# aymenboudhina/Multimodal_VQVAE_compression_audio_tactile

Measured on AMD Instinct MI355X. Metric: encode+VQ+decode token-frames/sec (1 frame = 13.33 ms of paired 24 kHz audio+tactile), higher is better.
Workload: dtype f32

## Files before the change

### multimodal_vqvae_compression_audio_tactile_amd/csrc/conv1d_mfma.hpp

```cpp
#pragma once
#include <hip/hip_runtime.h>
#include <stdio.h>
#include <stdlib.h>
#include <type_traits>
#include "det_math.hpp"
#include "kernels_small.hpp"

namespace mvq {

struct ConvArgs;
inline bool conv_dma_rows_ok(const ConvArgs& a);

__device__ __attribute__((aligned(16))) static const float g_zero16[4] = {0.0f, 0.0f, 0.0f, 0.0f};

int prof_begin(const char* kernel_name, double flops, hipStream_t s);
void prof_end(int idx, hipStream_t s);
bool prof_enabled();

typedef float f32x16 __attribute__((ext_vector_type(16)));
typedef float f32x4 __attribute__((ext_vector_type(4)));

struct ConvArgs {
    const float* x;
    const float* wp;
// ... 137 lines not shown
                     : "=&s"(keep) : "v"(off[0]), "v"(off[1]), "v"(off[2]), "v"(off[3]), "v"(off[4]), "v"(off[5]), "v"(off[6]), [base] "s"(base), [dst] "s"(dst), [inc] "n"(INC) : "memory", "scc");
    else
        asm volatile(MVQ_DMA_HEAD MVQ_DMAU_FIRST(1) MVQ_DMAU_NEXT(2) MVQ_DMAU_NEXT(3) MVQ_DMAU_NEXT(4) MVQ_DMAU_NEXT(5) MVQ_DMAU_NEXT(6) MVQ_DMAU_NEXT(7) MVQ_DMAU_NEXT(8) MVQ_DMA_TAIL
                     : "=&s"(keep) : "v"(off[0]), "v"(off[1]), "v"(off[2]), "v"(off[3]), "v"(off[4]), "v"(off[5]), "v"(off[6]), "v"(off[7]), [base] "s"(base), [dst] "s"(dst), [inc] "n"(INC) : "memory", "scc");
}
__device__ __forceinline__ void lds_dma_masked_uni(unsigned off, unsigned long long base, unsigned dst, unsigned long long mask)
{
    unsigned keep;
    unsigned long long keep_exec;
    asm volatile("s_mov_b64 %1, exec\n\ts_mov_b64 exec, %[mask]\n\t"
                 "s_mov_b32 %0, m0\n\ts_mov_b32 m0, %[dst]\n\ts_nop 0\n\tglobal_load_lds_dwordx4 %2, %[base]\n\ts_mov_b32 m0, %0\n\t"
                 "s_mov_b64 exec, %1"
                 : "=&s"(keep), "=&s"(keep_exec) : "v"(off), [base] "s"(base), [dst] "s"(dst), [mask] "s"(mask) : "memory");
}

__device__ __forceinline__ unsigned long long dma_scalar_base(const float* p)
{
    const unsigned long long v = (unsigned long long)p;
    const unsigned lo = __builtin_amdgcn_readfirstlane((unsigned)v), hi = __builtin_amdgcn_readfirstlane((unsigned)(v >> 32));
    unsigned long long s = ((unsigned long long)hi << 32) | lo;
    asm volatile("s_nop 4" : "+s"(s));
    return s;
}

template <int KS, int STRIDE, int DIL, int BM, int XP, int MT, int NT, int NS, int BASE = 0>
struct AsmOperandLoop {
    template <int S, int I>
    static __device__ __forceinline__ void load_a(float (&av)[MT], unsigned a_addr)
    {
        if constexpr (I < MT) {
            av[I] = lds_read_imm<BASE + (2 * S * BM + I * 32) * 4>(a_addr);
            load_a<S, I + 1>(av, a_addr);
        }
    }
    template <int S, int J>
    static __device__ __forceinline__ void load_b(float (&bv)[NT], unsigned b_same, unsigned b_cross)
    {
        if constexpr (J < NT) {
            constexpr int k0 = 2 * S;
            constexpr int off0 = (k0 / KS) * XP + (k0 % KS) * DIL;
            constexpr bool cross = ((k0 + 1) / KS) != (k0 / KS);
            bv[J] = lds_read_imm<BASE + (off0 + J * 32 * STRIDE) * 4>(cross ? b_cross : b_same);
            load_b<S, J + 1>(bv, b_same, b_cross);
        }
    }
    template <int S>
    static __device__ __forceinline__ void load_step(float (&av)[MT], float (&bv)[NT], unsigned a_addr, unsigned b_same, unsigned b_cross)
    {
        load_a<S, 0>(av, a_addr);
        load_b<S, 0>(bv, b_same, b_cross);
    }
    static __device__ __forceinline__ void mfma_step(f32x16_t (&acc)[MT][NT], const float (&av)[MT], const float (&bv)[NT])
    {
#pragma unroll
        for (int i = 0; i < MT; ++i)
#pragma unroll
            for (int j = 0; j < NT; ++j)
                acc[i][j] = __builtin_amdgcn_mfma_f32_32x32x2f32(av[i], bv[j], acc[i][j], 0, 0, 0);
    }
    template <int S>
    static __device__ __forceinline__ void run_from(f32x16_t (&acc)[MT][NT], float (&av0)[MT], float (&bv0)[NT], float (&av1)[MT],
                                                    float (&bv1)[NT], unsigned a_addr, unsigned b_same, unsigned b_cross)
    {
        if constexpr (S < NS) {
            if constexpr (S + 1 < NS) {
                if constexpr ((S + 1) % 2 == 0) load_step<S + 1>(av0, bv0, a_addr, b_same, b_cross);
                else load_step<S + 1>(av1, bv1, a_addr, b_same, b_cross);
            }
            constexpr int PW = (S + 1 < NS) ? MT + NT : 0;
            __builtin_amdgcn_sched_barrier(0);
            if constexpr (S % 2 == 0) lgkm_wait_step<PW, MT, NT>(av0, bv0);
            else lgkm_wait_step<PW, MT, NT>(av1, bv1);
            __builtin_amdgcn_sched_barrier(0);
            if constexpr (S % 2 == 0) mfma_step(acc, av0, bv0);
            else mfma_step(acc, av1, bv1);
            __builtin_amdgcn_sched_barrier(0);
            run_from<S + 1>(acc, av0, bv0, av1, bv1, a_addr, b_same, b_cross);
        }
    }
};

constexpr int cgcd(int a, int b) { return b == 0 ? a : cgcd(b, a % b); }

template <int KS, int STRIDE, int DIL, int CK, int MT, int NT, int WAVES_M, int WAVES_N, int UPS>
struct ConvCfg {
    static constexpr int BM = 32 * MT * WAVES_M;
    static constexpr int BN = 32 * NT * WAVES_N;
    static constexpr int KC = CK * KS;
    static constexpr int XT = (BN - 1) * STRIDE + (KS - 1) * DIL + 1;
    static constexpr bool XALIGNED = (KS == 1 && STRIDE == 1);
    static constexpr int XV = XALIGNED ? (XT + 3) / 4 : (XT + 3 + 3) / 4;
    static constexpr int XTP = XV * 4 + 4;
    static constexpr int W_FLOATS = KC * BM;
    static constexpr int X_FLOATS = CK * XTP;
    static constexpr int STAGE_FLOATS = 2 * (W_FLOATS + X_FLOATS);
    static constexpr int BNP = BN + 4;
    static constexpr int CT_FLOATS = BM * BNP;
    static constexpr int EH = ((UPS == 0 || 32 % (UPS ? UPS : 1) == 0) && MT % 2 == 0 && CT_FLOATS > STAGE_FLOATS) ? 2 : 1;
    static constexpr int CTH_FLOATS = CT_FLOATS / EH;
    static constexpr int QPR = BN / 4;
    static constexpr int CQ = cgcd(QPR, 64 * WAVES_M * WAVES_N);
    static constexpr int JN = QPR / CQ;
    static constexpr int RSTEP = (64 * WAVES_M * WAVES_N) / CQ;
    static constexpr bool REG_GEOM = (UPS == 0) && (32 % RSTEP == 0);
    static constexpr int TB_FLOATS = REG_GEOM ? 2 * BM : 0;
    static constexpr int EPI_FLOATS = CTH_FLOATS + TB_FLOATS;
    static constexpr int EPI_FLOATS_FUSE = CT_FLOATS + TB_FLOATS;
    static constexpr int LDS_FLOATS = STAGE_FLOATS > EPI_FLOATS ? STAGE_FLOATS : EPI_FLOATS;
    static constexpr bool FOUR_WAVES = WAVES_M * WAVES_N == 4;
    static constexpr bool RING_FITS = (size_t)3 * (KC * BM + CK * XV * 4) * 4 <= 64 * 1024;
    static constexpr int MIN_WPE = (FOUR_WAVES && LDS_FLOATS * 4 <= 53 * 1024 && !(WAVES_N == 4 && NT == 2) && RING_FITS && MT * NT <= 4) ? 3
                                                                                                                : (WAVES_M * WAVES_N) / 2;
    static constexpr int LDS_FLOATS_FUSE = STAGE_FLOATS > EPI_FLOATS_FUSE ? STAGE_FLOATS : EPI_FLOATS_FUSE;
    static constexpr int MIN_WPE_FUSE = (FOUR_WAVES && (LDS_FLOATS_FUSE + 5 * BM) * 4 * 3 <= 160 * 1024) ? 3 : (WAVES_M * WAVES_N) / 2;
    static constexpr int XV4 = XV * 4;
    static constexpr int DMA_STAGE_FLOATS = W_FLOATS + CK * XV4;
    static constexpr int DMA_NV = DMA_STAGE_FLOATS / 4;
    static constexpr int DMA_NU = (DMA_NV + 64 * WAVES_M * WAVES_N - 1) / (64 * WAVES_M * WAVES_N);
    static constexpr int LDS_FLOATS_DMA = 3 * DMA_STAGE_FLOATS > EPI_FLOATS ? 3 * DMA_STAGE_FLOATS : EPI_FLOATS;
    static constexpr int LDS_FLOATS_FUSE_DMA = 3 * DMA_STAGE_FLOATS > EPI_FLOATS_FUSE ? 3 * DMA_STAGE_FLOATS : EPI_FLOATS_FUSE;
    static constexpr int W_VEC = W_FLOATS / 4;
    static constexpr int NTHR = 64 * WAVES_M * WAVES_N;
    static constexpr int W_PER_THREAD = (W_VEC + NTHR - 1) / NTHR;
    static constexpr int XV_TOTAL = CK * XV;
    static constexpr int XV_PER_THREAD = (XV_TOTAL + NTHR - 1) / NTHR;
    static constexpr int XS_TOTAL = CK * XT;
    static constexpr int XS_PER_THREAD = (XS_TOTAL + NTHR - 1) / NTHR;
    static constexpr int XREGS = (4 * XV_PER_THREAD > XS_PER_THREAD) ? 4 * XV_PER_THREAD : XS_PER_THREAD;
    static_assert(WAVES_M * WAVES_N == 4 || WAVES_M * WAVES_N == 8, "block is 4 or 8 waves");
    static_assert(KC % 2 == 0, "chunk K must be even (32x32x2 MFMA)");
    static_assert(BM % 4 == 0, "float4 weight staging");
};

template <int KS, int STRIDE, int DIL, int CK, int MT, int NT, int WAVES_M, int WAVES_N, int UPS, bool VEC>
struct ConvTile {
    using C = ConvCfg<KS, STRIDE, DIL, CK, MT, NT, WAVES_M, WAVES_N, UPS>;
    const float* wp; const float* xb; const float* Al;
    float* Ws; float* Xs;
    int tid, Tin, Cin, Mpad, m0, t_in0, g_al;
    bool snake_in;

    __device__ __forceinline__ void load_chunk(int chunk, f32x4 (&wreg)[C::W_PER_THREAD], f32x4 (&xv)[C::XV_PER_THREAD], float (&xs)[C::XS_PER_THREAD]) const
    {
        const int ci0 = chunk * CK;
        const float* wsrc = wp + (size_t)ci0 * KS * Mpad + m0;
#pragma unroll
        for (int u = 0; u < C::W_PER_THREAD; ++u) {
            int v = tid + u * C::NTHR;
            if (C::W_VEC % C::NTHR != 0) v = v < C::W_VEC ? v : C::W_VEC - 1;
            const int row = v / (C::BM / 4);
            const int c4 = v - row * (C::BM / 4);
            wreg[u] = *reinterpret_cast<const f32x4*>(wsrc + (size_t)row * Mpad + c4 * 4);
        }
        if (VEC) {
#pragma unroll
            for (int u = 0; u < C::XV_PER_THREAD; ++u) {
                int e = tid + u * C::NTHR;
                if (C::XV_TOTAL % C::NTHR != 0) e = e < C::XV_TOTAL ? e : C::XV_TOTAL - 1;
                const int cl = e / C::XV;
                const int v = e - cl * C::XV;
                const int g = g_al + 4 * v;
                const bool ok = g >= 0 && g < Tin;
                const int gc = ok ? g : 0;
                xv[u] = *reinterpret_cast<const f32x4*>(xb + (size_t)(ci0 + cl) * Tin + gc);
            }
        } else {
#pragma unroll
            for (int u = 0; u < C::XS_PER_THREAD; ++u) {
                int e = tid + u * C::NTHR;
                if (C::XS_TOTAL % C::NTHR != 0) e = e < C::XS_TOTAL ? e : C::XS_TOTAL - 1;
                const int cl = e / C::XT;
                const int xi = e - cl * C::XT;
                const int g = t_in0 + xi;
                const bool ok = g >= 0 && g < Tin;
                const int gc = ok ? g : 0;
                xs[u] = xb[(size_t)(ci0 + cl) * Tin + gc];
            }
        }
    }

    __device__ __forceinline__ void store_chunk(int chunk, int buf, const f32x4 (&wreg)[C::W_PER_THREAD],
                                                const f32x4 (&xv)[C::XV_PER_THREAD],
                                                const float (&xs)[C::XS_PER_THREAD]) const
    {
        const int ci0 = chunk * CK;
        float* wdst = Ws + buf * C::W_FLOATS;
        float* xdst = Xs + buf * C::X_FLOATS;
#pragma unroll
        for (int u = 0; u < C::W_PER_THREAD; ++u) {
            const int v = tid + u * C::NTHR;
            if (C::W_VEC % C::NTHR == 0 || v < C::W_VEC) *reinterpret_cast<f32x4*>(wdst + v * 4) = wreg[u];
        }
        if (VEC) {
#pragma unroll
            for (int u = 0; u < C::XV_PER_THREAD; ++u) {
                const int e = tid + u * C::NTHR;
                const int ec = (C::XV_TOTAL % C::NTHR != 0 && e >= C::XV_TOTAL) ? C::XV_TOTAL - 1 : e;
                const int cl = ec / C::XV;
                const int v = ec - cl * C::XV;
                const int g = g_al + 4 * v;
                const bool ok = g >= 0 && g < Tin;
                f32x4 q = xv[u];
                if (!ok) q = f32x4{0.0f, 0.0f, 0.0f, 0.0f};
                if (snake_in) {
                    const float al = Al[ci0 + cl], inv = Al[Cin + ci0 + cl];
                    q.x = det_snake(q.x, al, inv); q.y = det_snake(q.y, al, inv);
                    q.z = det_snake(q.z, al, inv); q.w = det_snake(q.w, al, inv);
                }
                if (C::XV_TOTAL % C::NTHR == 0 || e < C::XV_TOTAL)
                    *reinterpret_cast<f32x4*>(xdst + cl * C::XTP + 4 * v) = q;
            }
        } else {
#pragma unroll
            for (int u = 0; u < C::XS_PER_THREAD; ++u) {
                const int e = tid + u * C::NTHR;
                const int ec = (C::XS_TOTAL % C::NTHR != 0 && e >= C::XS_TOTAL) ? C::XS_TOTAL - 1 : e;
                const int cl = ec / C::XT;
                const int xi = ec - cl * C::XT;
                const int g = t_in0 + xi;
                float q = (g >= 0 && g < Tin) ? xs[u] : 0.0f;
                if (snake_in) q = det_snake(q, Al[ci0 + cl], Al[Cin + ci0 + cl]);
                if (C::XS_TOTAL % C::NTHR == 0 || e < C::XS_TOTAL) xdst[cl * C::XTP + xi] = q;
            }
        }
    }
};

template <int KS, int STRIDE, int DIL, int CK, int MT, int NT, int WAVES_M, int WAVES_N, int UPS, bool VEC, bool FUSE>
__device__ __forceinline__ void conv1d_mfma_body(const ConvArgs& a)
{
    using C = ConvCfg<KS, STRIDE, DIL, CK, MT, NT, WAVES_M, WAVES_N, UPS>;
    extern __shared__ __attribute__((aligned(16))) float smem[];
    float* const Ws = smem;
    float* const Xs = smem + 2 * C::W_FLOATS;
    float* const Ep = smem + (FUSE ? (a.dma ? C::LDS_FLOATS_FUSE_DMA : C::LDS_FLOATS_FUSE) : (a.dma ? C::LDS_FLOATS_DMA : C::LDS_FLOATS));
    constexpr int EP_MID = 2;
    float* const Al = Ep + 3 * C::BM;

    const int tid = threadIdx.x;
    const int lane = tid & 63;
    const int wave = tid >> 6;
    const int wm = wave / WAVES_N;
    const int wn = wave % WAVES_N;
    const int l31 = lane & 31;
    const int h = lane >> 5;

    int bx = blockIdx.x, by = blockIdx.y;
    if (a.row_fast) {
        const int xcd = bx & 7, j = bx >> 3;
        by = j % a.row_fast;
        bx = (j / a.row_fast) * 8 + xcd;
        if (bx >= a.n_tiles * a.B) return;
    }
    const int b = bx / a.n_tiles;
    const int tile_n = bx - b * a.n_tiles;
    const int n0 = a.n_base + tile_n * C::BN;
    const int m0 = by * C::BM;
    const int t_in0 = n0 * STRIDE - a.pad;
    const int g_al = t_in0 & ~3;
    const int shift = VEC ? (t_in0 - g_al) : 0;
    const int Cin = a.Cin;
    const int n_chunks = Cin / CK;
    const bool snake_in = a.alpha_in != nullptr;

    if (snake_in) {
        for (int c = tid; c < Cin; c += C::NTHR) {
            const float al = a.alpha_in[c];
            Al[c] = al;
            Al[Cin + c] = 1.0f / (al + 1e-9f);
        }
    }
    for (int r = tid; r < C::BM; r += C::NTHR) {
        int m = m0 + r;
        m = m < a.Mrows ? m : a.Mrows - 1;
        const int ch = m / (UPS ? UPS : 1);
        const float* tabs[4] = {a.alpha_out, a.y2 ? a.alpha2 : nullptr, FUSE ? a.alpha_mid : (a.dsn_src ? a.dsn_alpha : nullptr), nullptr};
#pragma unroll
        for (int k = 0; k < 3; ++k) {
            Ep[k * C::BM + r] = tabs[k] ? 1.0f / (tabs[k][ch] + 1e-9f) : 1.0f;
        }
    }

    ConvTile<KS, STRIDE, DIL, CK, MT, NT, WAVES_M, WAVES_N, UPS, VEC> tile;
    tile.wp = a.wp; tile.xb = a.x + (size_t)b * Cin * a.Tin; tile.Al = Al; tile.Ws = Ws; tile.Xs = Xs;
    tile.tid = tid; tile.Tin = a.Tin; tile.Cin = Cin; tile.Mpad = a.Mpad; tile.m0 = m0; tile.t_in0 = t_in0;
    tile.g_al = g_al; tile.snake_in = snake_in;

    f32x16 acc[MT][NT];
#pragma unroll
    for (int i = 0; i < MT; ++i)
#pragma unroll
        for (int j = 0; j < NT; ++j)
#pragma unroll
            for (int r = 0; r < 16; ++r) acc[i][j][r] = 0.0f;

    f32x4 wreg[C::W_PER_THREAD];
    f32x4 xv[C::XV_PER_THREAD];
    float xs[C::XS_PER_THREAD];

    constexpr int D_SAME = DIL;
    constexpr int D_CROSS = C::XTP - (KS - 1) * DIL;
    const int a_base = h * C::BM + wm * (MT * 32) + l31;
    const int b_base = (wn * (NT * 32) + l31) * STRIDE + shift;
    const int b_same = b_base + h * D_SAME;
    const int b_cross = b_base + h * D_CROSS;

    constexpr int NS = C::KC / 2;
    auto mfma_chunk = [&](int buf) __attribute__((always_inline)) {
        const float* wsrc = Ws + buf * C::W_FLOATS + a_base;
        const float* xs_same = Xs + buf * C::X_FLOATS + b_same;
        const float* xs_cross = Xs + buf * C::X_FLOATS + b_cross;
        float av[2][MT], bv[2][NT];
        auto load_step = [&](int st, int pb) __attribute__((always_inline)) {
            const int k0 = 2 * st;
            const int off0 = (k0 / KS) * C::XTP + (k0 % KS) * DIL;
            const bool cross = ((k0 + 1) / KS) != (k0 / KS);
            const float* xsp = cross ? xs_cross : xs_same;
#pragma unroll
            for (int i = 0; i < MT; ++i) av[pb][i] = wsrc[k0 * C::BM + i * 32];
#pragma unroll
            for (int j = 0; j < NT; ++j) bv[pb][j] = xsp[off0 + j * 32 * STRIDE];
        };
        load_step(0, 0);
#pragma unroll
        for (int s = 0; s < NS; ++s) {
            const int pb = s & 1;
            if (s + 1 < NS) load_step(s + 1, (s + 1) & 1);
#pragma unroll
            for (int i = 0; i < MT; ++i)
#pragma unroll
                for (int j = 0; j < NT; ++j)
                    acc[i][j] = __builtin_amdgcn_mfma_f32_32x32x2f32(av[pb][i], bv[pb][j], acc[i][j], 0, 0, 0);
            __builtin_amdgcn_sched_group_barrier(0x100, MT + NT, 0);
            __builtin_amdgcn_sched_group_barrier(0x008, MT * NT, 0);
        }
    };

    constexpr bool DMA_FITS = FUSE ? ((size_t)C::LDS_FLOATS_FUSE_DMA + 3 * C::BM) * 4 * 2 <= 160 * 1024 : (size_t)C::LDS_FLOATS_DMA * 4 <= 64 * 1024;
    bool use_dma = false;
    if constexpr (VEC && DMA_FITS) use_dma = a.dma != 0;
    if (use_dma) {
      if constexpr (VEC && DMA_FITS) {
        constexpr int NU = C::DMA_NU;
        constexpr int XP = C::XV4;
        constexpr int D_CROSS_D = XP - (KS - 1) * DIL;
        const int bd_same = b_base + h * D_SAME;
        const int bd_cross = b_base + h * D_CROSS_D;
        const unsigned lds0 = (unsigned)(size_t)smem;
        const int wave_u = __builtin_amdgcn_readfirstlane(wave);
        using AL = AsmOperandLoop<KS, STRIDE, DIL, C::BM, XP, MT, NT, NS>;
        auto chunk_rt = [&](int stage, auto&& issue) __attribute__((always_inline)) {
            const unsigned sb = lds0 + (unsigned)(stage * C::DMA_STAGE_FLOATS * 4);
            const unsigned a_addr = sb + (unsigned)(a_base * 4);
            const unsigned b_s = sb + (unsigned)((C::W_FLOATS + bd_same) * 4), b_c = sb + (unsigned)((C::W_FLOATS + bd_cross) * 4);
            float av0[MT], bv0[NT], av1[MT], bv1[NT];
            AL::template load_step<0>(av0, bv0, a_addr, b_s, b_c);
            issue();
            AL::template run_from<0>(acc, av0, bv0, av1, bv1, a_addr, b_s, b_c);
        };
        constexpr int NW = WAVES_M * WAVES_N;
        constexpr int XPC = CK * C::XV;
        constexpr int WI_W = (C::W_VEC + 63) / 64, WI_X = (XPC + 63) / 64;
// ... 72 lines not shown
                    st_n2 = st_n2 == 2 ? 0 : st_n2 + 1;
                }
            };
            dma_uni(0);
            if (n_chunks > 1) dma_uni(1);
            const int my_issue = (WI_W - wave_u + NW - 1) / NW + (WI_X - xw + NW - 1) / NW;
            if ((WI_W + WI_X) % NW != 0 && my_issue > NI_MIN) k_loop_uni(std::integral_constant<int, NI_MIN + 1>{});
            else k_loop_uni(std::integral_constant<int, NI_MIN>{});
          }
        } else {
        const float* src[NU];
        bool live[NU];
        long long step_b[NU];
#pragma unroll
        for (int u = 0; u < NU; ++u) {
            const int p = tid + u * C::NTHR;
            live[u] = p < C::DMA_NV;
            if (p < C::W_VEC) {
                const int row = p / (C::BM / 4), c4 = p - row * (C::BM / 4);
                src[u] = a.wp + (size_t)row * a.Mpad + m0 + c4 * 4;
                step_b[u] = (long long)CK * KS * a.Mpad;
            } else {
                const int q = (p < C::DMA_NV ? p : C::DMA_NV - 1) - C::W_VEC;
                const int cl = q / C::XV, v = q - cl * C::XV;
                const int g = g_al + 4 * v;
                bool ok = g >= 0 && g < a.Tin;
                const float* sp = tile.xb + (size_t)cl * a.Tin + g;
                long long st = (long long)CK * a.Tin;
                if (a.vp_seg) {
                    const int gg = ok ? g : 0;
                    const int seg = (int)__umulhi((unsigned)gg, a.vp_magic_in), pos = gg - seg * a.vp_per_in;
                    const int item = b * a.vp_seg + seg;
                    ok = ok && pos < a.vp_valid_in && item < a.vp_btrue;
                    sp = a.x + ((size_t)(ok ? item : 0) * a.Cin + cl) * a.vp_tin_phys + (ok ? pos : 0);
                    st = (long long)CK * a.vp_tin_phys;
                }
                src[u] = ok ? sp : g_zero16;
                step_b[u] = ok ? st : 0;
            }
        }
        const int n_issue = (NU - 1) * C::NTHR + wave_u * 64 < C::DMA_NV ? NU : NU - 1;
        constexpr int NFULL = C::DMA_NV / C::NTHR < NU ? C::DMA_NV / C::NTHR : NU;
        auto dma_chunk = [&](int stage) __attribute__((always_inline)) {
            const unsigned dst0 = lds0 + (unsigned)(stage * C::DMA_STAGE_FLOATS * 4) + (unsigned)(wave_u * 64 * 16);
            if constexpr (NFULL > 0) lds_dma_burst<NFULL, C::NTHR * 16>(src, dst0);
#pragma unroll
            for (int u = NFULL; u < NU; ++u) {
                if (live[u]) lds_dma_burst<1, C::NTHR * 16>(src + u, dst0 + (unsigned)(u * C::NTHR * 16));
            }
#pragma unroll
            for (int u = 0; u < NU; ++u) src[u] += step_b[u];
        };
        dma_chunk(0);
        if (n_chunks > 1) dma_chunk(1);
        int st_c = 0, st_n2 = 2;
        for (int c = 0; c < n_chunks; ++c) {
            if (c + 1 >= n_chunks) asm volatile("s_waitcnt vmcnt(0)" ::: "memory");
            else if (n_issue == NU) asm volatile("s_waitcnt vmcnt(%0)" :: "n"(NU) : "memory");
            else asm volatile("s_waitcnt vmcnt(%0)" :: "n"(NU - 1) : "memory");
            __syncthreads();
            chunk_rt(st_c, [&]() __attribute__((always_inline)) { if (c + 2 < n_chunks) dma_chunk(st_n2); });
            st_c = st_c == 2 ? 0 : st_c + 1;
            st_n2 = st_n2 == 2 ? 0 : st_n2 + 1;
        }
        }
      }
    } else {
    tile.load_chunk(0, wreg, xv, xs);
    __syncthreads();
    tile.store_chunk(0, 0, wreg, xv, xs);
    __syncthreads();
    for (int c = 0; c + 1 < n_chunks; ++c) {
        tile.load_chunk(c + 1, wreg, xv, xs);
        __builtin_amdgcn_sched_barrier(0);
        mfma_chunk(c & 1);
        __builtin_amdgcn_sched_barrier(0);
        tile.store_chunk(c + 1, (c + 1) & 1, wreg, xv, xs);
        __syncthreads();
    }
    mfma_chunk((n_chunks - 1) & 1);
    }

    const float* ep_bias = a.bias;
    if (FUSE) {
        float* const Ht = smem;
        __syncthreads();
#pragma unroll
        for (int i = 0; i < MT; ++i)
#pragma unroll
            for (int r = 0; r < 16; ++r) {
                const int row = (wm * MT + i) * 32 + (r & 3) + 8 * (r >> 2) + 4 * h;
                const float bv = a.bias ? a.bias[row] : 0.0f;
                const float al = a.alpha_mid[row], inv = Ep[EP_MID * C::BM + row];
#pragma unroll
                for (int j = 0; j < NT; ++j) {
                    Ht[row * C::BNP + (wn * NT + j) * 32 + l31] = det_snake(acc[i][j][r] + bv, al, inv);
                    acc[i][j][r] = 0.0f;
                }
            }
        __syncthreads();
        constexpr int K2 = C::BM / 2;
        constexpr int G = 8;
        static_assert(K2 % G == 0, "BM must be a multiple of 16");
        const float* w2 = a.w2p + (size_t)h * a.Mpad + wm * (MT * 32) + l31;
        const float* hsrc = Ht + h * C::BNP + wn * (NT * 32) + l31;
        float aw[2][G][MT];
#pragma unroll
        for (int g = 0; g < G; ++g)
#pragma unroll
            for (int i = 0; i < MT; ++i) aw[0][g][i] = w2[(size_t)(2 * g) * a.Mpad + i * 32];
#pragma unroll
        for (int grp = 0; grp < K2 / G; ++grp) {
            if (grp + 1 < K2 / G) {
#pragma unroll
                for (int g = 0; g < G; ++g)
#pragma unroll
                    for (int i = 0; i < MT; ++i)
                        aw[(grp + 1) & 1][g][i] = w2[(size_t)(2 * ((grp + 1) * G + g)) * a.Mpad + i * 32];
            }
#pragma unroll
            for (int g = 0; g < G; ++g) {
                const int s2 = grp * G + g;
                float bvv[NT];
#pragma unroll
                for (int j = 0; j < NT; ++j) bvv[j] = hsrc[2 * s2 * C::BNP + j * 32];
#pragma unroll
                for (int i = 0; i < MT; ++i)
#pragma unroll
                    for (int j = 0; j < NT; ++j)
                        acc[i][j] = __builtin_amdgcn_mfma_f32_32x32x2f32(aw[grp & 1][g][i], bvv[j], acc[i][j], 0, 0, 0);
            }
        }
        ep_bias = a.bias2;
    }

    const bool has_res = (UPS == 0) && a.residual != nullptr;
    const bool snake_out = a.alpha_out != nullptr;
    const bool do_tanh = a.act == 1;
    const bool do_gelu = a.act == 2;
    const bool direct = (UPS != 0) && (C::BM % (UPS ? UPS : 1) != 0);
    if (direct) {
#pragma unroll
        for (int i = 0; i < MT; ++i) {
#pragma unroll
            for (int r = 0; r < 16; ++r) {
                const int row = (r & 3) + 8 * (r >> 2) + 4 * h;
                const int m = m0 + (wm * MT + i) * 32 + row;
                const bool mok = m < a.Mrows;
                const int mc = mok ? m : a.Mrows - 1;
                const int co = mc / (UPS ? UPS : 1), rr = mc - co * (UPS ? UPS : 1);
                const float bv = ep_bias ? ep_bias[co] : 0.0f;
                const int lr = (wm * MT + i) * 32 + row;
                const float al = snake_out ? a.alpha_out[co] : 1.0f, inv = Ep[lr];
                const size_t rowoff = ((size_t)b * a.Cout + co) * a.Tout;
#pragma unroll
                for (int j = 0; j < NT; ++j) {
                    const int n = n0 + (wn * NT + j) * 32 + l31;
                    int t = n * (UPS ? UPS : 1) + rr - a.up_p;
                    bool ok = mok && n < a.Ncols && t >= 0 && (a.up_per_out ? true : t < a.Tout);
                    t = ok ? t : 0;
                    size_t ro = rowoff;
                    if (a.up_per_out) {
                        const int sg = (int)__umulhi((unsigned)t, a.up_magic);
                        t -= sg * a.up_per_out;
                        const int bb = b * a.up_seg + sg;
                        ok = ok && t < a.up_valid_out && bb < a.up_btrue;
                        ro = ((size_t)(ok ? bb : 0) * a.Cout + co) * a.Tout;
                        t = ok ? t : 0;
                    }
                    float v = acc[i][j][r] + bv;
                    const bool tail = a.tvalid && t >= a.tvalid;
                    if (ok && a.y2) a.y2[ro + t] = tail ? 0.0f : det_snake(v, a.alpha2[co], Ep[C::BM + lr]);
                    if (snake_out) v = det_snake(v, al, inv);
                    if (ok) a.y[ro + t] = tail ? 0.0f : v;
                }
            }
        }
        return;
    }

    float* const Ct = smem;
    constexpr int EHP = FUSE ? 1 : C::EH;
    constexpr int MTH = MT / EHP;
    constexpr int BMH = C::BM / EHP;
    auto tile_row_of = [&](int lrow, int pass) __attribute__((always_inline)) {
        if (EHP == 1) return lrow;
        const int g = lrow >> 5;
        return ((g / MTH) * MT + pass * MTH + (g % MTH)) * 32 + (lrow & 31);
    };
    auto epilogue_pass = [&](auto HP) __attribute__((always_inline)) {
    constexpr int hp = decltype(HP)::value;
    __syncthreads();
#pragma unroll
    for (int il = 0; il < MTH; ++il)
#pragma unroll
        for (int r = 0; r < 16; ++r) {
            const int row = (wm * MTH + il) * 32 + (r & 3) + 8 * (r >> 2) + 4 * h;
#pragma unroll
            for (int j = 0; j < NT; ++j) Ct[row * C::BNP + (wn * NT + j) * 32 + l31] = acc[hp * MTH + il][j][r];
        }
    constexpr int NVQ = BMH * C::BN / 4;
    constexpr bool PRE_RES = (UPS == 0) && (NVQ % C::NTHR == 0) && (NVQ / C::NTHR <= 16);
    constexpr int RES_IT = PRE_RES ? NVQ / C::NTHR : 1;
    constexpr int CQ = C::CQ, JN = C::JN;
    constexpr bool REG = PRE_RES && C::REG_GEOM && (BMH % C::RSTEP == 0);
    constexpr int RSTEP = REG ? C::RSTEP : 1;
    const bool reg_ok = REG && !(a.y2 && a.alpha_out);
    const int q_c0 = REG ? tid % CQ : 0, q_r0 = REG ? tid / CQ : 0;
    auto reg_k = [&](int it, int pass) __attribute__((always_inline)) {
        const int lr = (it / JN) * RSTEP;
        if (EHP == 1) return lr;
        const int g = lr >> 5;
        return ((g / MTH) * MT + pass * MTH + (g % MTH)) * 32 + (lr & 31);
    };
    const size_t blk_off = a.vp_seg ? ((size_t)b * a.vp_seg * a.Cout + m0) * a.Tout : ((size_t)b * a.Cout + m0) * a.Tout + n0;
    const unsigned q_t0 = (unsigned)(q_r0 * a.Tout);
    bool q_nok[JN];
    unsigned q_col[JN];
    int q_vpos[JN];
#pragma unroll
    for (int j = 0; j < JN; ++j) {
        const int n = n0 + 4 * (q_c0 + j * CQ);
        q_nok[j] = n < a.Ncols;
        q_col[j] = 4u * (q_c0 + j * CQ);
        q_vpos[j] = 0;
        if (a.vp_seg) {
            const int nn = q_nok[j] ? n : 0;
            const int seg = (int)__umulhi((unsigned)nn, a.vp_magic_out), pos = nn - seg * a.vp_per_out;
            q_nok[j] = q_nok[j] && b * a.vp_seg + seg < a.vp_btrue && pos < a.Tout;
            q_col[j] = (unsigned)(seg * a.Cout * a.Tout + pos);
            q_vpos[j] = pos;
        }
    }
    f32x4 res_q[RES_IT];
    if (PRE_RES && has_res && a.ovec4) {
        bool pre_done = false;
        if constexpr (REG) if (reg_ok) {
            pre_done = true;
            const float* resb = a.residual + blk_off;
#pragma unroll
            for (int it = 0; it < RES_IT; ++it) {
                const int k = reg_k(it, hp), j = it % JN;
                const bool ok = q_nok[j] && m0 + q_r0 + k < a.Mrows;
                res_q[it] = *reinterpret_cast<const f32x4*>(resb + (ok ? q_t0 + (unsigned)(k * a.Tout) + q_col[j] : 0u));
            }
        }
        if (!pre_done) {
#pragma unroll
            for (int it = 0; it < RES_IT; ++it) {
                const int e = tid + it * C::NTHR;
                const int row = e / (C::BN / 4);
                const int c4 = e - row * (C::BN / 4);
                const int m = m0 + tile_row_of(row, hp), n = n0 + 4 * c4;
                const bool ok = m < a.Mrows && n < a.Ncols;
                const size_t off = ((size_t)b * a.Cout + (ok ? m : 0)) * a.Tout + (ok ? n : 0);
                res_q[it] = *reinterpret_cast<const f32x4*>(a.residual + off);
            }
        }
    }
    float* const Tb = smem + (FUSE ? C::CT_FLOATS : C::CTH_FLOATS);
    if (reg_ok && hp == 0) {
        const float* const ax = a.y2 ? a.alpha2 : a.alpha_out;
        for (int r = tid; r < C::BM; r += C::NTHR) {
            int m = m0 + r;
            m = m < a.Mrows ? m : a.Mrows - 1;
            Tb[r] = ep_bias ? ep_bias[m] : 0.0f;
            Tb[C::BM + r] = ax ? ax[m] : 1.0f;
        }
    }
    __syncthreads();
    auto tile_row = [&](int lrow) __attribute__((always_inline)) { return tile_row_of(lrow, hp); };

    if (UPS == 0) {
        if (a.ovec4) {
            constexpr int NV = BMH * C::BN / 4;
            auto quad = [&](int e, int it) __attribute__((always_inline)) {
                const int row = e / (C::BN / 4);
                const int c4 = e - row * (C::BN / 4);
                const int m = m0 + tile_row(row), n = n0 + 4 * c4;
                if (m < a.Mrows && n < a.Ncols) {
                    const float bv = ep_bias ? ep_bias[m] : 0.0f;
                    f32x4 v = *reinterpret_cast<const f32x4*>(Ct + row * C::BNP + 4 * c4);
                    const size_t off = ((size_t)b * a.Cout + m) * a.Tout + n;
                    v.x = v.x + bv; v.y = v.y + bv; v.z = v.z + bv; v.w = v.w + bv;
                    if (a.dsn_src) {
                        const float ad = a.dsn_alpha[m], id = Ep[2 * C::BM + tile_row(row)];
                        const f32x4 sv = *reinterpret_cast<const f32x4*>(a.dsn_src + off);
                        v.x = v.x * det_dsnake(sv.x, ad, id); v.y = v.y * det_dsnake(sv.y, ad, id);
                        v.z = v.z * det_dsnake(sv.z, ad, id); v.w = v.w * det_dsnake(sv.w, ad, id);
                    }
                    if (has_res) {
                        const f32x4 rv = PRE_RES ? res_q[PRE_RES ? it : 0] : *reinterpret_cast<const f32x4*>(a.residual + off);
                        v.x = v.x + rv.x; v.y = v.y + rv.y; v.z = v.z + rv.z; v.w = v.w + rv.w;
                    }
                    int nz = (a.tvalid && n + 4 > a.tvalid) ? n + 4 - a.tvalid : 0;
                    if (a.tper) {
                        const int nn = n - (int)__umulhi((unsigned)n, a.tper_magic) * a.tper;
                        nz = nn + 4 > a.tper_valid ? (nn >= a.tper_valid ? 4 : nn + 4 - a.tper_valid) : 0;
                    }
                    if (a.y2) {
                        const float a2 = a.alpha2[m], i2 = Ep[C::BM + tile_row(row)];
                        f32x4 w = {det_snake(v.x, a2, i2), det_snake(v.y, a2, i2), det_snake(v.z, a2, i2), det_snake(v.w, a2, i2)};
                        if (nz > 0) { w.w = 0.0f; if (nz > 1) w.z = 0.0f; if (nz > 2) w.y = 0.0f; if (nz > 3) w.x = 0.0f; }
                        *reinterpret_cast<f32x4*>(a.y2 + off) = w;
                    }
                    if (snake_out) {
                        const float al = a.alpha_out[m], inv = Ep[tile_row(row)];
                        v.x = det_snake(v.x, al, inv); v.y = det_snake(v.y, al, inv);
                        v.z = det_snake(v.z, al, inv); v.w = det_snake(v.w, al, inv);
                    }
                    if (do_tanh) { v.x = det_tanh(v.x); v.y = det_tanh(v.y); v.z = det_tanh(v.z); v.w = det_tanh(v.w); }
                    if (do_gelu) { v.x = det_gelu(v.x); v.y = det_gelu(v.y); v.z = det_gelu(v.z); v.w = det_gelu(v.w); }
                    if (nz > 0) { v.w = 0.0f; if (nz > 1) v.z = 0.0f; if (nz > 2) v.y = 0.0f; if (nz > 3) v.x = 0.0f; }
                    *reinterpret_cast<f32x4*>(a.y + off) = v;
                }
            };
            bool quads_done = false;
            if constexpr (REG) if (reg_ok) {
                quads_done = true;
                int nz[JN];
#pragma unroll
                for (int j = 0; j < JN; ++j) {
                    const int n = n0 + 4 * (q_c0 + j * CQ);
                    nz[j] = (a.tvalid && n + 4 > a.tvalid) ? n + 4 - a.tvalid : 0;
                    if (a.tper) {
                        const int nn = n - (int)__umulhi((unsigned)n, a.tper_magic) * a.tper;
                        nz[j] = nn + 4 > a.tper_valid ? (nn >= a.tper_valid ? 4 : nn + 4 - a.tper_valid) : 0;
                    }
                    if (a.vp_seg) {
                        const int pp = q_vpos[j];
                        nz[j] = pp + 4 > a.vp_valid_out ? (pp >= a.vp_valid_out ? 4 : pp + 4 - a.vp_valid_out) : 0;
                    }
                }
                float* const yb = a.y + blk_off;
                float* const y2b = a.y2 ? a.y2 + blk_off : nullptr;
                const float* const dsb = a.dsn_src ? a.dsn_src + blk_off : nullptr;
                const float* const ctq = Ct + q_r0 * C::BNP + 4 * q_c0;
                const float* const tbq = Tb + q_r0;
                const float* const epq = Ep + q_r0;
                auto reg_quads = [&](auto MODE_) __attribute__((always_inline)) {
                    constexpr int MODE = decltype(MODE_)::value;
                    const bool f_dsn = MODE == 0 ? (a.dsn_src != nullptr) : false;
                    const bool f_res = MODE == 0 ? has_res : (MODE == 1 || MODE == 2 || MODE == 5);
// ... 355 lines not shown
```

### multimodal_vqvae_compression_audio_tactile_amd/csrc/conv_ru.hip

```cpp
#include "conv_dispatch.hpp"
namespace mvq {
template <int DIL>
static hipError_t ru(const ConvArgs& a, int c, hipStream_t s)
{
    const long wide_blocks = (long)a.B * ((a.Ncols + (c == 64 ? 191 : 127)) / (c == 64 ? 192 : 128));
    const bool narrow = wide_blocks < 200 && !a.name_out;
    switch (c) {
        case 128: return narrow ? launch_residual_unit<DIL, 4, 2, 1, 2, 2>(a, s) : launch_residual_unit<DIL, 4, 1, 3, 4, 1>(a, s);
        case 96:  return launch_residual_unit<DIL, 4, 3, 1, 1, 4>(a, s);
        case 64:  return narrow ? launch_residual_unit<DIL, 8, 2, 1, 1, 4>(a, s) : launch_residual_unit<DIL, 4, 1, 3, 2, 2>(a, s);
    }
    return hipErrorInvalidValue;
}
hipError_t launch_residual_unit_fused(const ConvArgs& a, int dil, hipStream_t s)
{
    switch (dil) {
        case 1: return ru<1>(a, a.Cout, s);
        case 3: return ru<3>(a, a.Cout, s);
        case 9: return ru<9>(a, a.Cout, s);
    }
    return hipErrorInvalidValue;
}
}
```

Baseline: 61430.

## Keep fused residual-unit intermediate in registers via permlane swap and second MFMA

For fused residual-unit kernels with a single wave row (WAVES_M==1), the first conv's accumulators get bias and snake applied in registers. The lanes are then rearranged with permlane32_swap and fed straight into a second 32x32x2 MFMA pass against the 1x1 weights, streamed from global memory. This removes the LDS round-trip and barriers for the intermediate tile. It also lets the fused epilogue use the half-tile LDS split. A new dispatch path picks a 4-row-tile, 1x4-wave configuration for large 128-channel non-dilation-9 layers, trading more register pressure and different occupancy for less LDS traffic.

```diff
diff --git a/multimodal_vqvae_compression_audio_tactile_amd/csrc/conv1d_mfma.hpp b/multimodal_vqvae_compression_audio_tactile_amd/csrc/conv1d_mfma.hpp
--- a/multimodal_vqvae_compression_audio_tactile_amd/csrc/conv1d_mfma.hpp
+++ b/multimodal_vqvae_compression_audio_tactile_amd/csrc/conv1d_mfma.hpp
@@ -243,6 +243,15 @@
 
 constexpr int cgcd(int a, int b) { return b == 0 ? a : cgcd(b, a % b); }
 
+template <int FROM, int TO, class F>
+__device__ __forceinline__ void static_for(F&& f)
+{
+    if constexpr (FROM < TO) {
+        f(std::integral_constant<int, FROM>{});
+        static_for<FROM + 1, TO>(f);
+    }
+}
+
 template <int KS, int STRIDE, int DIL, int CK, int MT, int NT, int WAVES_M, int WAVES_N, int UPS>
 struct ConvCfg {
     static constexpr int BM = 32 * MT * WAVES_M;
@@ -266,20 +275,23 @@
     static constexpr bool REG_GEOM = (UPS == 0) && (32 % RSTEP == 0);
     static constexpr int TB_FLOATS = REG_GEOM ? 2 * BM : 0;
     static constexpr int EPI_FLOATS = CTH_FLOATS + TB_FLOATS;
-    static constexpr int EPI_FLOATS_FUSE = CT_FLOATS + TB_FLOATS;
+    static constexpr bool FUSE_REG = WAVES_M == 1;
+    static constexpr int EH_FUSE = FUSE_REG ? EH : 1;
+    static constexpr int MID_FLOATS = FUSE_REG ? 2 * BM : 0;
+    static constexpr int EPI_FLOATS_FUSE = CT_FLOATS / EH_FUSE + TB_FLOATS;
     static constexpr int LDS_FLOATS = STAGE_FLOATS > EPI_FLOATS ? STAGE_FLOATS : EPI_FLOATS;
     static constexpr bool FOUR_WAVES = WAVES_M * WAVES_N == 4;
     static constexpr bool RING_FITS = (size_t)3 * (KC * BM + CK * XV * 4) * 4 <= 64 * 1024;
     static constexpr int MIN_WPE = (FOUR_WAVES && LDS_FLOATS * 4 <= 53 * 1024 && !(WAVES_N == 4 && NT == 2) && RING_FITS && MT * NT <= 4) ? 3
                                                                                                                 : (WAVES_M * WAVES_N) / 2;
-    static constexpr int LDS_FLOATS_FUSE = STAGE_FLOATS > EPI_FLOATS_FUSE ? STAGE_FLOATS : EPI_FLOATS_FUSE;
+    static constexpr int LDS_FLOATS_FUSE = STAGE_FLOATS + MID_FLOATS > EPI_FLOATS_FUSE ? STAGE_FLOATS + MID_FLOATS : EPI_FLOATS_FUSE;
     static constexpr int MIN_WPE_FUSE = (FOUR_WAVES && (LDS_FLOATS_FUSE + 5 * BM) * 4 * 3 <= 160 * 1024) ? 3 : (WAVES_M * WAVES_N) / 2;
     static constexpr int XV4 = XV * 4;
     static constexpr int DMA_STAGE_FLOATS = W_FLOATS + CK * XV4;
     static constexpr int DMA_NV = DMA_STAGE_FLOATS / 4;
     static constexpr int DMA_NU = (DMA_NV + 64 * WAVES_M * WAVES_N - 1) / (64 * WAVES_M * WAVES_N);
     static constexpr int LDS_FLOATS_DMA = 3 * DMA_STAGE_FLOATS > EPI_FLOATS ? 3 * DMA_STAGE_FLOATS : EPI_FLOATS;
-    static constexpr int LDS_FLOATS_FUSE_DMA = 3 * DMA_STAGE_FLOATS > EPI_FLOATS_FUSE ? 3 * DMA_STAGE_FLOATS : EPI_FLOATS_FUSE;
+    static constexpr int LDS_FLOATS_FUSE_DMA = 3 * DMA_STAGE_FLOATS + MID_FLOATS > EPI_FLOATS_FUSE ? 3 * DMA_STAGE_FLOATS + MID_FLOATS : EPI_FLOATS_FUSE;
     static constexpr int W_VEC = W_FLOATS / 4;
     static constexpr int NTHR = 64 * WAVES_M * WAVES_N;
     static constexpr int W_PER_THREAD = (W_VEC + NTHR - 1) / NTHR;
@@ -397,14 +409,16 @@
     float* const Ep = smem + (FUSE ? (a.dma ? C::LDS_FLOATS_FUSE_DMA : C::LDS_FLOATS_FUSE) : (a.dma ? C::LDS_FLOATS_DMA : C::LDS_FLOATS));
     constexpr int EP_MID = 2;
     float* const Al = Ep + 3 * C::BM;
-
-    const int tid = threadIdx.x;
-    const int lane = tid & 63;
-    const int wave = tid >> 6;
+    constexpr bool FUSE_REG = FUSE && C::FUSE_REG;
+    float* const Mt = smem + (a.dma ? 3 * C::DMA_STAGE_FLOATS : C::STAGE_FLOATS);
+
+    int tid = threadIdx.x;
+    int lane = tid & 63;
+    int wave = tid >> 6;
     const int wm = wave / WAVES_N;
-    const int wn = wave % WAVES_N;
-    const int l31 = lane & 31;
-    const int h = lane >> 5;
+    int wn = wave % WAVES_N;
+    int l31 = lane & 31;
+    int h = lane >> 5;
 
     int bx = blockIdx.x, by = blockIdx.y;
     if (a.row_fast) {
@@ -413,9 +427,9 @@
         bx = (j / a.row_fast) * 8 + xcd;
         if (bx >= a.n_tiles * a.B) return;
     }
-    const int b = bx / a.n_tiles;
+    int b = bx / a.n_tiles;
     const int tile_n = bx - b * a.n_tiles;
-    const int n0 = a.n_base + tile_n * C::BN;
+    int n0 = a.n_base + tile_n * C::BN;
     const int m0 = by * C::BM;
     const int t_in0 = n0 * STRIDE - a.pad;
     const int g_al = t_in0 & ~3;
@@ -439,6 +453,10 @@
 #pragma unroll
         for (int k = 0; k < 3; ++k) {
             Ep[k * C::BM + r] = tabs[k] ? 1.0f / (tabs[k][ch] + 1e-9f) : 1.0f;
+        }
+        if constexpr (FUSE_REG) {
+            Mt[2 * r] = a.bias ? a.bias[ch] : 0.0f;
+            Mt[2 * r + 1] = a.alpha_mid[ch];
         }
     }
 
@@ -677,7 +695,72 @@
     }
 
     const float* ep_bias = a.bias;
-    if (FUSE) {
+    if constexpr (FUSE_REG) {
+        constexpr int K2 = C::BM / 2;
+        constexpr int G = MT > 3 ? 2 : 4;
+        constexpr int OG = (MT > 3 && MT % 2 == 0) ? 2 : MT;
+        constexpr int NGRP = K2 / G, NSTEP = (MT / OG) * NGRP;
+        static_assert(K2 % G == 0 && MT % OG == 0, "whole register groups, whole passes");
+        const unsigned wl = (unsigned)(h * C::BM + l31);
+        float aw[2][G][OG];
+        auto load_aw = [&](auto ST_) __attribute__((always_inline)) {
+            constexpr int ST = decltype(ST_)::value, pass = ST / NGRP, grp = ST % NGRP;
+#pragma unroll
+            for (int g = 0; g < G; ++g)
+#pragma unroll
+                for (int io = 0; io < OG; ++io)
+                    aw[ST & 1][g][io] = (a.w2p + 2 * (grp * G + g) * C::BM + (pass * OG + io) * 32)[wl];
+        };
+        load_aw(std::integral_constant<int, 0>{});
+        const float* const mt = Mt + 2 * 4 * h;
+        const float* const mi = Ep + EP_MID * C::BM + 4 * h;
+#pragma unroll
+        for (int i = 0; i < MT; ++i)
+#pragma unroll
+            for (int r = 0; r < 16; ++r) {
+                const int row = i * 32 + (r & 3) + 8 * (r >> 2);
+                const float bv = mt[2 * row], al = mt[2 * row + 1], inv = mi[row];
+#pragma unroll
+                for (int j = 0; j < NT; ++j) acc[i][j][r] = det_snake(acc[i][j][r] + bv, al, inv);
+            }
+#pragma unroll
+        for (int i = 0; i < MT; ++i)
+#pragma unroll
+            for (int j = 0; j < NT; ++j)
+#pragma unroll
+                for (int r = 0; r < 16; r += 2) {
+                    const auto sw = __builtin_amdgcn_permlane32_swap(__float_as_uint(acc[i][j][r]), __float_as_uint(acc[i][j][r + 1]), false, false);
+                    acc[i][j][r] = __uint_as_float(sw[0]);
+                    acc[i][j][r + 1] = __uint_as_float(sw[1]);
+                }
+        f32x16 out[MT][NT];
+#pragma unroll
+        for (int i = 0; i < MT; ++i)
+#pragma unroll
+            for (int j = 0; j < NT; ++j)
+#pragma unroll
+                for (int r = 0; r < 16; ++r) out[i][j][r] = 0.0f;
+        static_for<0, NSTEP>([&](auto ST_) __attribute__((always_inline)) {
+            constexpr int ST = decltype(ST_)::value, pass = ST / NGRP, grp = ST % NGRP;
+            if constexpr (ST + 1 < NSTEP) load_aw(std::integral_constant<int, ST + 1>{});
+#pragma unroll
+            for (int g = 0; g < G; ++g) {
+                const int s2 = grp * G + g, ci = s2 / 16, t = s2 % 4, rb = 4 * ((s2 % 16) / 4) + ((t & 1) << 1 | (t >> 1));
+#pragma unroll
+                for (int io = 0; io < OG; ++io)
+#pragma unroll
+                    for (int j = 0; j < NT; ++j)
+                        out[pass * OG + io][j] = __builtin_amdgcn_mfma_f32_32x32x2f32(aw[ST & 1][g][io], acc[ci][j][rb], out[pass * OG + io][j], 0, 0, 0);
+            }
+        });
+#pragma unroll
+        for (int i = 0; i < MT; ++i)
+#pragma unroll
+            for (int j = 0; j < NT; ++j) acc[i][j] = out[i][j];
+        ep_bias = a.bias2;
+        asm volatile("" : "+v"(tid), "+v"(b), "+v"(n0));
+        lane = tid & 63; wave = tid >> 6; wn = wave % WAVES_N; l31 = lane & 31; h = lane >> 5;
+    } else if (FUSE) {
         float* const Ht = smem;
         __syncthreads();
 #pragma unroll
@@ -775,7 +858,7 @@
     }
 
     float* const Ct = smem;
-    constexpr int EHP = FUSE ? 1 : C::EH;
+    constexpr int EHP = FUSE ? C::EH_FUSE : C::EH;
     constexpr int MTH = MT / EHP;
     constexpr int BMH = C::BM / EHP;
     auto tile_row_of = [&](int lrow, int pass) __attribute__((always_inline)) {
@@ -853,7 +936,7 @@
             }
         }
     }
-    float* const Tb = smem + (FUSE ? C::CT_FLOATS : C::CTH_FLOATS);
+    float* const Tb = smem + C::CT_FLOATS / EHP;
     if (reg_ok && hp == 0) {
         const float* const ax = a.y2 ? a.alpha2 : a.alpha_out;
         for (int r = tid; r < C::BM; r += C::NTHR) {
diff --git a/multimodal_vqvae_compression_audio_tactile_amd/csrc/conv_ru.hip b/multimodal_vqvae_compression_audio_tactile_amd/csrc/conv_ru.hip
--- a/multimodal_vqvae_compression_audio_tactile_amd/csrc/conv_ru.hip
+++ b/multimodal_vqvae_compression_audio_tactile_amd/csrc/conv_ru.hip
@@ -1,12 +1,18 @@
 #include "conv_dispatch.hpp"
 namespace mvq {
+static constexpr long RU128_SQUARE_MIN_BLOCKS = 2048;
 template <int DIL>
 static hipError_t ru(const ConvArgs& a, int c, hipStream_t s)
 {
     const long wide_blocks = (long)a.B * ((a.Ncols + (c == 64 ? 191 : 127)) / (c == 64 ? 192 : 128));
     const bool narrow = wide_blocks < 200 && !a.name_out;
     switch (c) {
-        case 128: return narrow ? launch_residual_unit<DIL, 4, 2, 1, 2, 2>(a, s) : launch_residual_unit<DIL, 4, 1, 3, 4, 1>(a, s);
+        case 128:
+            if (narrow) return launch_residual_unit<DIL, 4, 2, 1, 2, 2>(a, s);
+            if constexpr (DIL != 9) {
+                if (wide_blocks >= RU128_SQUARE_MIN_BLOCKS) return launch_residual_unit<DIL, 4, 4, 1, 1, 4>(a, s);
+            }
+            return launch_residual_unit<DIL, 4, 1, 3, 4, 1>(a, s);
         case 96:  return launch_residual_unit<DIL, 4, 3, 1, 1, 4>(a, s);
         case 64:  return narrow ? launch_residual_unit<DIL, 8, 2, 1, 1, 4>(a, s) : launch_residual_unit<DIL, 4, 1, 3, 2, 2>(a, s);
     }
```

Result: no change. 61810, median of 6 (+0.6%).
